# thedonutfactory/zig-tfhe

Measured on AMD Instinct MI355X. Metric: gate-bootstraps/sec (NAND, 128-bit params) at 1/2/4/8 MI355X; % HBM roofline, higher is better.
Workload: dtype f64; 1 GPU; 1024 NAND gate bootstraps per GPU per step, SECURITY_128_BIT (n=700, N=1024, L=3, Bg=2^6, t=9); global_batch=1024, params=128, parallelism=dp1

## Files before the change

include/tfhe_gpu.h:

```cpp
#ifndef TFHE_GPU_H
#define TFHE_GPU_H

#include <stddef.h>
#include <stdint.h>

#ifdef __cplusplus
extern "C" {
#endif

#define TFHE_GPU_ABI_VERSION 7

enum {
    TFHE_OK = 0,
    TFHE_ERR_INVALID = -1,
    TFHE_ERR_HIP = -2,
    TFHE_ERR_NO_KEY = -3,
    TFHE_ERR_OOM = -4,
    TFHE_ERR_IO = -5,
    TFHE_ERR_DEVICE = -6
};

enum {
    TFHE_GATE_NAND = 0, TFHE_GATE_OR = 1, TFHE_GATE_AND = 2, TFHE_GATE_XOR = 3,
    TFHE_GATE_XNOR = 4, TFHE_GATE_NOR = 5, TFHE_GATE_ANDNY = 6, TFHE_GATE_ANDYN = 7,
// ... 44 lines not shown
    TFHE_OPT_KS_NARROW = 4,
    TFHE_OPT_KS_ITEM_GROUPS = 5,
    TFHE_OPT_KS_SEL_ITEMS = 6,
    TFHE_OPT_CIRCUIT_PACK = 7,
    TFHE_OPT_TWIDDLES = 8,
    TFHE_OPT_ARITH = 9,
    TFHE_OPT_BR_SYNC = 10,
    TFHE_OPT_BR_SPIN_CAP = 11,
    TFHE_OPT_HOST_PIPELINE = 12,
    TFHE_OPT_CIRCUIT_SPLIT = 13,
    TFHE_OPT_FUSED_ADMITTED = 14,
    TFHE_OPT_LEVEL_ISSUE_US = 15,
    TFHE_OPT_KEY_ROW_RMS_PPM = 16,
    TFHE_OPT_HOST_STAGING = 17,
    TFHE_OPT_CMUX_FORM = 18,
    TFHE_OPT_PACK_SCRATCH_MB = 19
};
enum { TFHE_STAGING_PAGEABLE = 0, TFHE_STAGING_PINNED = 1 };
enum { TFHE_ARITH_AUTO = 0, TFHE_ARITH_REFERENCE = 1, TFHE_ARITH_FUSED_FORCED = 2 };
enum { TFHE_TWIDDLES_GLIBC = 0, TFHE_TWIDDLES_FDLIBM = 1 };
int tfhe_gpu_set_option(tfhe_gpu_ctx *ctx, int key, int64_t value);
int tfhe_gpu_get_option(const tfhe_gpu_ctx *ctx, int key, int64_t *value);
const char *tfhe_gpu_last_kernels(tfhe_gpu_ctx *ctx);
int tfhe_fft_tables(uint32_t N, int source, double *twist_re, double *twist_im, double *stage_re,
                    double *stage_im);

int tfhe_gpu_load_cloud_key(tfhe_gpu_ctx *ctx, uint32_t decomposition_offset,
                            const uint32_t *testvec_a, const uint32_t *testvec_b,
                            const double *bsk, size_t bsk_len,
                            const uint32_t *ksk, size_t ksk_len);
int tfhe_gpu_keygen(tfhe_gpu_ctx *ctx, uint64_t secret_seed, uint64_t cloud_seed,
// ... 204 lines not shown
```

zig-tfhe_amd/csrc/tfhe_gpu.cpp:

```cpp
#include "tfhe_gpu.h"

#include <algorithm>
#include <cmath>
#include <cstdio>
#include <cstring>
#include <string>
#include <vector>

#include "host_math.hpp"
#include "tfhe_ctx.hpp"

using namespace tfhe;

namespace tfhe {

static thread_local std::string g_create_error;
static int create_fail(int code, const std::string &msg) {
    g_create_error = msg;
    return code;
}

int ensure(Device &d, DevBuf &b, size_t bytes) {
    if (b.bytes >= bytes) return TFHE_OK;
    b.bytes = 0;
// ... 40 lines not shown
    }
    return TFHE_OK;
}

int ks_gemm_args(Device &d, size_t B, KsGemm &G) {
    G = KsGemm();
    if (!ks_use_gemm(d.opts, d.K.iks_t, d.K.basebit, B, nullptr)) return TFHE_OK;
    if (!d.d_ksk_gemm) {
        hipError_t e = hipMalloc((void **)d.d_ksk_gemm.make(d.device), ks_gemm_bytes(d.K, 1024, d.K.iks_t, d.K.basebit));
        if (e != hipSuccess) return fail(d, TFHE_ERR_OOM, "hipMalloc(ksk gemm layout)");
    }
    if (!d.ksk_gemm_ok) {
        HIPCHK(d, launch_ksk_to_gemm(d.K, d.d_ksk, d.d_ksk_gemm, 1024, d.K.iks_t, d.K.basebit, d.stream));
        d.ksk_gemm_ok = true;
    }
    int rc = ensure(d, d.s_kspart, ks_gemm_part_bytes(d.K, B, 1024, d.K.basebit));
    if (rc) return rc;
    G.kg = d.d_ksk_gemm;
    G.part = d.s_kspart.as<uint32_t>();
    return TFHE_OK;
}

static int ensure_tie_flags(Device &d, size_t B) {
    if (d.s_ties.bytes >= B) return TFHE_OK;
    int rc = ensure(d, d.s_ties, B);
    if (rc) return rc;
    HIPCHK(d, hipMemsetAsync(d.s_ties.p, 0, d.s_ties.bytes, d.stream));
    return TFHE_OK;
}

int run_bootstrap_dev(Device &d, const uint8_t *ops, const uint32_t *a, const uint32_t *b,
                      const uint32_t *testvec_dev, uint32_t *out, size_t B, int kind, const uint32_t *idx,
                      const uint32_t *tv_sel) {
    const bool key_switch = kind == RUN_BOOTSTRAP;
// ... 426 lines not shown
    if (!rc) rc = ensure(d, d.s_a, B * wb);
    if (!rc && b) rc = ensure(d, d.s_b, B * wb);
    if (!rc) rc = ensure(d, d.s_out, B * wb);
    if (!rc) rc = ensure(d, d.s_lv1, B * 1025 * sizeof(uint32_t));
    if (!rc) rc = ensure_tie_flags(d, B);
    if (rc) return rc;
    if (!d.pipe_ev) HIPCHK(d, hipEventCreateWithFlags(d.pipe_ev.make(d.device), hipEventDisableTiming));
    for (Stream &p : d.pipe)
        if (!p) HIPCHK(d, hipStreamCreateWithFlags(p.make(d.device), hipStreamNonBlocking));
    if (!d.workers) d.workers.reset(new WorkerPool(PIPE_STREAMS));
    KsGemm G;
    rc = ks_gemm_args(d, chunk, G);
    if (rc) return rc;
    std::vector<KsGemm> Gs(S, G);
    if (G.kg) {
        const size_t pb = ks_gemm_part_bytes(d.K, chunk, 1024, d.K.basebit);
        rc = ensure(d, d.s_kspart, pb * S);
        if (rc) return rc;
        for (int s = 0; s < S; s++) Gs[s].part = (uint32_t *)(d.s_kspart.as<char>() + (size_t)s * pb);
    }
    HIPCHK(d, hipEventRecord(d.pipe_ev, d.stream));
    LaunchOpts o = d.opts;
    if (!o.br_form) o.br_form = 1;
    char *pin_ops = d.pin_in.p, *pin_a = pin_ops + ops_bytes, *pin_b = pin_a + a_bytes;
    uint8_t *d_ops = d.s_ops.as<uint8_t>();
    uint32_t *d_a = d.s_a.as<uint32_t>(), *d_b = d.s_b.as<uint32_t>(), *d_out = d.s_out.as<uint32_t>();
    uint32_t *d_lv1 = d.s_lv1.as<uint32_t>();
    std::vector<hipError_t> err(S, hipSuccess);
    std::vector<const char *> where(S, "");
    d.workers->run(S, [&](int s) {
        hipStream_t st = d.pipe[s];
// ... 125 lines not shown
static int reencrypt_on(Device &d, const tfhe_gpu_reenc_key &key, size_t slot, const uint32_t *in, uint32_t *out,
                        size_t B, bool dev = false) {
    const tfhe_gpu_reenc_key::Copy &k = key.dev[slot];
    if (k.device != d.device) return fail(d, TFHE_ERR_INVALID, "key belongs to another device");
    if (B == 0) return TFHE_OK;
    HIPCHK(d, hipSetDevice(d.device));
    const size_t w = tlwe0_words(d.P);
    Io io{d, dev};
    int rc = ensure(d, d.s_a, B * w * 4 + KS_GEMM_INPUT_SLACK);
    if (!rc) rc = io.out(out, B * w * 4);
    if (rc) return rc;
    if (dev) HIPCHK(d, hipMemcpyAsync(d.s_a.p, in, B * w * 4, hipMemcpyDeviceToDevice, d.stream));
    else if ((rc = h2d(d, d.s_a, in, B * w * 4))) return rc;
    KsGemm G;
    if (k.key_gemm) {
        rc = ensure(d, d.s_kspart, ks_gemm_part_bytes(d.K, B, (int)d.P.n, (int)key.basebit));
        if (rc) return rc;
        G.kg = k.key_gemm;
        G.part = d.s_kspart.as<uint32_t>();
    }
    HIPCHK(d, launch_reencrypt(d.K, (int)key.t, (int)key.basebit, d.s_a.as<const uint32_t>(), k.key, out, B, d.stream,
                               d.opts, &d.last_ks, &G));
    return io.finish();
}

}

extern "C" int tfhe_circuit_schedule(size_t n_inputs, size_t n_gates, const uint8_t *ops, const uint32_t *in_a,
                                     const uint32_t *in_b, uint32_t cus, int pack, uint32_t *levels, uint32_t *depth) {
    if ((n_gates && (!ops || !in_a || !in_b || !levels)) || cus == 0) return TFHE_ERR_INVALID;
    if (n_inputs + n_gates > 0xFFFFFFFFull) return TFHE_ERR_INVALID;
// ... 233 lines not shown
    case TFHE_OPT_BR_SYNC:
        ok = v == 1;
        if (!ok) why = "option " + std::to_string(key) + ": only 1 (the variant with value 0 was removed in round 5)";
        break;
    case TFHE_OPT_KS_NARROW:
    case TFHE_OPT_CIRCUIT_PACK: ok = v == 0 || v == 1; break;
    case TFHE_OPT_KS_ITEM_GROUPS: ok = v == 0 || v == 1 || v == 2 || v == 4 || v == 8; break;
    case TFHE_OPT_KS_SEL_ITEMS: ok = v == 8 || v == 16 || v == 32; break;
    case TFHE_OPT_ARITH: ok = v == TFHE_ARITH_AUTO || v == TFHE_ARITH_REFERENCE || v == TFHE_ARITH_FUSED_FORCED; break;
    case TFHE_OPT_BR_SPIN_CAP: ok = v >= 0 && v <= 0xFFFFFFFFll; break;
    case TFHE_OPT_HOST_PIPELINE: ok = v == 0 || v == 1; break;
    case TFHE_OPT_CIRCUIT_SPLIT: ok = v >= 0 && v <= 2; break;
    case TFHE_OPT_HOST_STAGING: ok = v == TFHE_STAGING_PAGEABLE || v == TFHE_STAGING_PINNED; break;
    case TFHE_OPT_CMUX_FORM: ok = v >= 0 && v <= 2; break;
    case TFHE_OPT_PACK_SCRATCH_MB: ok = v >= 1 && v <= 256; break;
    case TFHE_OPT_TWIDDLES:
        ok = v == TFHE_TWIDDLES_GLIBC || v == TFHE_TWIDDLES_FDLIBM;
        if (ok && d.key_from_keygen && v != d.twiddle_source) {
            why = "TFHE_OPT_TWIDDLES: the resident key was generated (tfhe_gpu_keygen) with the current FFT tables; "
                  "set the twiddle source before keygen";
            return false;
        }
        break;
    default: why = "unknown option key " + std::to_string(key); return false;
    }
    if (!ok && why.empty()) why = "bad value " + std::to_string(v) + " for option " + std::to_string(key);
    return ok;
}

static int apply_option(Device &d, int key, int64_t v) {
// ... 1 lines not shown
    switch (key) {
    case TFHE_OPT_BR_FORM: o.br_form = (int)v; break;
    case TFHE_OPT_BR_LOADER: break;
    case TFHE_OPT_KS_FORM: o.ks_form = (int)v; break;
    case TFHE_OPT_KS_NARROW: o.ks_narrow = (int)v; break;
    case TFHE_OPT_KS_ITEM_GROUPS: o.ks_groups = (int)v; break;
    case TFHE_OPT_KS_SEL_ITEMS: o.ks_sel_items = (int)v; break;
    case TFHE_OPT_CIRCUIT_PACK: d.circuit_pack = v; break;
    case TFHE_OPT_TWIDDLES: return v == d.twiddle_source ? TFHE_OK : build_tables(d, (int)v);
    case TFHE_OPT_BR_SYNC: break;
    case TFHE_OPT_ARITH: o.arith_strict = v == TFHE_ARITH_REFERENCE ? 1 : v == TFHE_ARITH_FUSED_FORCED ? 2 : 0; break;
    case TFHE_OPT_BR_SPIN_CAP: d.K.spin_cap = (uint32_t)v; break;
    case TFHE_OPT_HOST_PIPELINE: d.pipeline = v; break;
    case TFHE_OPT_CMUX_FORM: o.cmux_form = (int)v; break;
    case TFHE_OPT_PACK_SCRATCH_MB: d.pack_scratch_mb = v; break;
    case TFHE_OPT_HOST_STAGING:
        if (d.stage_used) HIPCHK(d, hipStreamSynchronize(d.stream));
        d.stage_used = 0;
        d.host_staging = v;
        break;
    default: return TFHE_ERR_INVALID;
    }
    return TFHE_OK;
}

}

extern "C" {

int tfhe_gpu_set_option(tfhe_gpu_ctx *c, int key, int64_t v) {
// ... 21 lines not shown
    case TFHE_OPT_KS_ITEM_GROUPS: *v = o.ks_groups; break;
    case TFHE_OPT_KS_SEL_ITEMS: *v = o.ks_sel_items; break;
    case TFHE_OPT_CIRCUIT_PACK: *v = d.circuit_pack; break;
    case TFHE_OPT_TWIDDLES: *v = d.twiddle_source; break;
    case TFHE_OPT_ARITH: *v = o.arith_strict == 1 ? TFHE_ARITH_REFERENCE : o.arith_strict == 2 ? TFHE_ARITH_FUSED_FORCED : TFHE_ARITH_AUTO; break;
    case TFHE_OPT_FUSED_ADMITTED: *v = o.key_fused_ok; break;
    case TFHE_OPT_LEVEL_ISSUE_US: *v = c->level_issue_us; break;
    case TFHE_OPT_KEY_ROW_RMS_PPM: *v = (int64_t)std::llround(d.bk_row_rms * 1e6); break;
    case TFHE_OPT_BR_SYNC: *v = 1; break;
    case TFHE_OPT_BR_SPIN_CAP: *v = d.K.spin_cap; break;
    case TFHE_OPT_HOST_PIPELINE: *v = d.pipeline; break;
    case TFHE_OPT_CIRCUIT_SPLIT: *v = c->circuit_split; break;
    case TFHE_OPT_HOST_STAGING: *v = d.host_staging; break;
    case TFHE_OPT_CMUX_FORM: *v = o.cmux_form; break;
    case TFHE_OPT_PACK_SCRATCH_MB: *v = d.pack_scratch_mb; break;
    default: return TFHE_ERR_INVALID;
    }
    return TFHE_OK;
}

const char *tfhe_gpu_last_kernels(tfhe_gpu_ctx *c) {
    if (!c) return "";
    const Device &d = c->dev[0];
    c->last_kernels = d.last_br;
    if (d.last_ks && d.last_ks[0]) c->last_kernels += std::string(" + ") + d.last_ks;
    return c->last_kernels.c_str();
}


int tfhe_gpu_create_multi(const tfhe_params *params, int num_devices, const int *devices, tfhe_gpu_ctx **out) {
// ... 180 lines not shown
```

zig-tfhe_amd/csrc/tfhe_internal.hpp:

```cpp
#pragma once

#include <hip/hip_runtime.h>

#include <cstddef>
#include <cstdint>

namespace tfhe {

struct C2 {
    double x, y;
};

struct KParams {
    int n;
    int N;
    int L;
    int bgbit;
    int basebit;
    int iks_t;
    uint32_t offset;
    int ks_stride;
    uint32_t *err;
    uint32_t spin_cap;
    uint8_t *tie_flags;
// ... 17 lines not shown
    BR_OUT_LV0_EXTRACT2 = 2,
};

struct DevTables {
    const C2 *twist;
    const C2 *tw;
    C2 twa[4];
};

struct LaunchOpts {
    int br_form = 0;
    int ks_form = 3;
    int ks_narrow = 0;
    int ks_groups = 0;
    int ks_sel_items = 8;
    int arith_strict = 0;
    int key_fused_ok = 1;
    int cmux_form = 0;
};
inline bool fused_allowed(const LaunchOpts &O) {
    return O.arith_strict == 2 || (O.arith_strict == 0 && O.key_fused_ok != 0);
}

#if defined(TFHE_PHASE_PROF) && !defined(TFHE_AB_BUILD)
#define TFHE_AB_BUILD 1
#endif
bool kernels_ab_build();
bool ab_forms_linked();

struct BrBatch {
// ... 17 lines not shown
struct BrGeometry {
    dim3 grid, block;
};
BrGeometry br_geometry(char form, size_t B);
hipError_t launch_br(const BrEntry &k, const BrGeometry &g, const KParams &P, const DevTables &T, const BrBatch &b,
                     hipStream_t s, const char **used);
hipError_t launch_blind_rotate(const KParams &P, const DevTables &T, const BrBatch &b, hipStream_t s,
                               const LaunchOpts &O = LaunchOpts(), const char **used = nullptr);
size_t device_cus();
double blind_rotate_cost(size_t B, size_t cus, int L = 3);
hipError_t launch_tlwe_gather(const KParams &P, const uint32_t *src, const uint32_t *idx, uint32_t *dst,
                              size_t count, bool negate, hipStream_t s);
struct KsGemm {
    const uint32_t *kg = nullptr;
    uint32_t *part = nullptr;
};
size_t ks_gemm_bytes(const KParams &P, int n_in, int t, int basebit);
size_t ks_gemm_part_bytes(const KParams &P, size_t B, int n_in, int basebit);
bool ks_gemm_supported(int t, int basebit);
bool ks_use_gemm(const LaunchOpts &O, int t, int basebit, size_t B, const KsGemm *G);
constexpr size_t KS_GEMM_INPUT_SLACK = 16;
hipError_t launch_ksk_to_gemm(const KParams &P, const uint32_t *ksk, uint32_t *kg, int n_in, int t, int basebit,
                              hipStream_t s);
hipError_t launch_key_switch(const KParams &P, const uint32_t *lv1, const uint32_t *ksk,
                             uint32_t *out, size_t B, hipStream_t s, const LaunchOpts &O = LaunchOpts(),
                             const char **used = nullptr, const KsGemm *G = nullptr);
struct PackSums {
    int splits = 0;
    uint32_t bias = 0;
};
size_t pack_gemm_bytes(const KParams &P, int t, int basebit);
size_t pack_gemm_part_bytes(const KParams &P, size_t items, int basebit);
hipError_t launch_pack_key_to_gemm(const KParams &P, const uint32_t *rows, uint32_t *kg, int t, int basebit,
// ... 62 lines not shown
```

zig-tfhe_amd/csrc/tfhe_kernels.hip:

```cpp
#include <algorithm>
#include <string>
#include <type_traits>

#include "tfhe_device.hpp"

namespace tfhe {


constexpr int BO_GATES = 8;
constexpr int BO_LDS_BUF = 2048 * 4;
constexpr int BO_LDS_AT = 1024 * 2;
constexpr int BO_LDS_TOTAL = BR_LDS_BK + BR_LDS_TW + BR_LDS_TWIST + BO_GATES * (BO_LDS_BUF + BO_LDS_AT);
static_assert(BO_LDS_TOTAL <= 160 * 1024, "octo form LDS");
constexpr int BO_LDS_BUF_AT = BR_LDS_BK + BR_LDS_TW + BR_LDS_TWIST;
static_assert(BO_LDS_BUF_AT % 4096 == 0 && BO_LDS_BUF % 4096 == 0, "gather_rot needs 4 KB-aligned buffers");

DEV void issue_bk_pair_async512(const double2 *__restrict__ src, double2 *slot, int tid) {
    const uint32_t base = (uint32_t)(size_t)(lds_void_t *)slot + (uint32_t)(tid & ~63) * 16;
    const uint32_t voff = (uint32_t)tid * 16;
#pragma unroll
    for (int k = 0; k < 4; k++) {
        const uint32_t dst = __builtin_amdgcn_readfirstlane(base + 512 * 16 * k);
        const double2 *piece = src + 512 * k;
        uint32_t keep;
// ... 533 lines not shown
            (w < out_w && i < n_in) ? ksk[((size_t)(base * t) * i + (size_t)base * j + k) * rs + w] : 0u;
        v |= (((word >> (8 * b)) & 255u) ^ 128u) << (8 * e4);
    }
    kg[x] = v;
}

template <int N>
DEV void kg_wait() {
    static_assert(N >= 0 && N <= 15, "kg_wait");
#define KG_W(n_) if constexpr (N == n_) asm volatile("s_waitcnt vmcnt(" #n_ ")" ::: "memory");
    KG_W(0) KG_W(1) KG_W(2) KG_W(3) KG_W(4) KG_W(5) KG_W(6) KG_W(7)
    KG_W(8) KG_W(9) KG_W(10) KG_W(11) KG_W(12) KG_W(13) KG_W(14) KG_W(15)
#undef KG_W
}

template <int T, int BASEBIT>
__global__ __launch_bounds__(64 * KG_WAVES, 1) void k_key_switch_gemm(KParams P, const uint32_t *__restrict__ lv1,
                                                                   const uint32_t *__restrict__ kg,
                                                                   uint32_t *__restrict__ part, size_t B,
                                                                   int ib_per_split, int n_in, int in_stride,
                                                                   int out_w) {
    constexpr int CB = BASEBIT == 2 ? 8 : 4;
    constexpr int KS = BASEBIT == 2 ? 1 : 4;
    constexpr int STEP_BYTES = KS * 4 * 1024;
    constexpr int WORDS_BYTES = CB * KG_ITEMS * 4;
    constexpr int WORD_DMAS = CB / 4;
    constexpr int BUF_BYTES = T * STEP_BYTES + WORDS_BYTES;
    constexpr int STAGES = 3 * BUF_BYTES <= 160 * 1024 ? 3 : 2;
    constexpr int LOADER_DMAS = T * KS + WORD_DMAS;
    constexpr int OTHER_DMAS = WORD_DMAS;
    static_assert(STAGES * BUF_BYTES <= 160 * 1024, "gemm key-switch LDS");
    __shared__ __attribute__((aligned(16))) unsigned char smem[STAGES * BUF_BYTES];
    const int tid = threadIdx.x, lane = tid & 63;
    const int v = __builtin_amdgcn_readfirstlane(tid >> 6);
    const bool loader = v < 4;
    const int w32 = (out_w + 31) / 32;
    const int wt = blockIdx.x;
    const int nib = kg_blocks(n_in, BASEBIT);
    const int ib_lo = blockIdx.z * ib_per_split, ib_hi = min(nib, ib_lo + ib_per_split);
    const size_t m_wg = (size_t)blockIdx.y * KG_ITEMS;
    const int h = lane >> 5, c = lane & 31;
    const uint32_t *a_src[WORD_DMAS];
#pragma unroll
    for (int r = 0; r < WORD_DMAS; r++) {
        const size_t m = m_wg + (CB == 8 ? 256 * r + (tid >> 1) : tid);
        a_src[r] = lv1 + (m < B ? m : B - 1) * (size_t)in_stride + (CB == 8 ? 4 * (tid & 1) : 0);
    }
    const uint32_t lds0 = (uint32_t)(size_t)(lds_void_t *)smem;
    auto issue = [&](int ib, int slot) {
        const uint32_t base = lds0 + slot * BUF_BYTES;
        if (loader) {
#pragma unroll
            for (int j = 0; j < T; j++)
#pragma unroll
                for (int st = 0; st < KS; st++) {
                    const uint32_t *src = kg + ((((size_t)j * nib + ib) * w32 + wt) * KS + st) * 1024 + tid * 4;
                    const uint32_t dst =
                        __builtin_amdgcn_readfirstlane(base + j * STEP_BYTES + st * 4096 + (tid & ~63) * 16);
                    uint32_t keep;
                    asm volatile(
                        "s_mov_b32 %0, m0\n\ts_mov_b32 m0, %2\n\ts_nop 0\n\tglobal_load_lds_dwordx4 %1, off\n\ts_mov_b32 m0, %0"
                        : "=&s"(keep)
                        : "v"(src), "s"(dst)
                        : "memory");
                }
        }
#pragma unroll
        for (int r = 0; r < WORD_DMAS; r++) {
            const uint32_t dst =
                __builtin_amdgcn_readfirstlane(base + T * STEP_BYTES + r * 256 * 32 + (tid & ~63) * 16);
            uint32_t keep;
            asm volatile(
                "s_mov_b32 %0, m0\n\ts_mov_b32 m0, %2\n\ts_nop 0\n\tglobal_load_lds_dwordx4 %1, off\n\ts_mov_b32 m0, %0"
                : "=&s"(keep)
                : "v"(a_src[r] + CB * ib), "s"(dst)
                : "memory");
        }
    };
    kg_v16i acc[2][4];
#pragma unroll
    for (int s = 0; s < 2; s++)
#pragma unroll
        for (int b = 0; b < 4; b++) acc[s][b] = kg_v16i{};
    const uint32_t prec = 1u << (32 - (1 + BASEBIT * T));
#pragma unroll
    for (int k = 0; k < STAGES - 1; k++)
        if (ib_lo + k < ib_hi) issue(ib_lo + k, k);
    for (int ib = ib_lo; ib < ib_hi; ib++) {
        const int slot = (ib - ib_lo) % STAGES;
        const int ahead = min(STAGES - 2, ib_hi - 1 - ib);
        if (ahead == 1) {
            if (loader) kg_wait<LOADER_DMAS>();
            else kg_wait<OTHER_DMAS>();
        } else {
            kg_wait<0>();
        }
        __syncthreads();
        if (ib + STAGES - 1 < ib_hi) issue(ib + STAGES - 1, (slot + STAGES - 1) % STAGES);
        const unsigned char *buf = smem + slot * BUF_BYTES;
        const uint32_t *words = reinterpret_cast<const uint32_t *>(buf + T * STEP_BYTES);
        if constexpr (BASEBIT == 2) {
            uint32_t pk[2][4];
#pragma unroll
            for (int s = 0; s < 2; s++) {
                const kg_v4i wv = *reinterpret_cast<const kg_v4i *>(words + (64 * v + 32 * s + c) * 8 + 4 * h);
#pragma unroll
                for (int q = 0; q < 4; q++) pk[s][q] = ((uint32_t)wv[q] + prec) >> (32 - 2 * T);
            }
#pragma unroll
            for (int j = 0; j < T; j++) {
                kg_v4i a[2];
#pragma unroll
                for (int s = 0; s < 2; s++)
#pragma unroll
                    for (int q = 0; q < 4; q++)
                        a[s][q] = (int)(1u << (8u * ((pk[s][q] >> (2 * (T - 1 - j))) & 3u)));
#pragma unroll
                for (int b = 0; b < 4; b++) {
                    const kg_v4i bf = *reinterpret_cast<const kg_v4i *>(buf + j * STEP_BYTES + b * 1024 + lane * 16);
#pragma unroll
                    for (int s = 0; s < 2; s++)
                        acc[s][b] = __builtin_amdgcn_mfma_i32_32x32x32_i8(a[s], bf, acc[s][b], 0, 0, 0);
                }
            }
        } else {
            uint32_t pk[2][4];
#pragma unroll
            for (int s = 0; s < 2; s++) {
                const kg_v4i wv = *reinterpret_cast<const kg_v4i *>(words + (64 * v + 32 * s + c) * 4);
#pragma unroll
                for (int q = 0; q < 4; q++) pk[s][q] = ((uint32_t)wv[q] + prec) >> (32 - BASEBIT * T);
            }
#pragma unroll
            for (int j = 0; j < T; j++)
#pragma unroll
                for (int st = 0; st < KS; st++) {
                    kg_v4i a[2];
#pragma unroll
// ... 4 lines not shown
#pragma unroll
                        for (int q = 0; q < 4; q++) a[s][q] = word == q ? (int)one : 0;
                    }
#pragma unroll
                    for (int b = 0; b < 4; b++) {
                        const kg_v4i bf = *reinterpret_cast<const kg_v4i *>(buf + j * STEP_BYTES + st * 4096 +
                                                                            b * 1024 + lane * 16);
#pragma unroll
                        for (int s = 0; s < 2; s++)
                            acc[s][b] = __builtin_amdgcn_mfma_i32_32x32x32_i8(a[s], bf, acc[s][b], 0, 0, 0);
                    }
                }
        }
    }
    const int n1 = out_w;
    uint32_t *pz = part + (size_t)blockIdx.z * B * n1;
    const int w = 32 * wt + c;
    const size_t m_base = m_wg + 64 * v;
#pragma unroll
    for (int s = 0; s < 2; s++)
#pragma unroll
        for (int reg = 0; reg < 16; reg++) {
            const size_t m = m_base + 32 * s + (reg & 3) + 8 * (reg >> 2) + 4 * h;
            const uint32_t val = (uint32_t)acc[s][0][reg] + ((uint32_t)acc[s][1][reg] << 8) +
                                 ((uint32_t)acc[s][2][reg] << 16) + ((uint32_t)acc[s][3][reg] << 24);
            if (m < B && w < n1) pz[m * n1 + w] = val;
        }
}

__global__ void k_ks_gemm_reduce(KParams P, const uint32_t *__restrict__ lv1, const uint32_t *__restrict__ part,
                                 uint32_t *__restrict__ out, size_t B, int splits, int n_in, int in_stride, int t,
// ... 662 lines not shown
        }))
        return true;
    if (gw == 4 && basebit == 5 && B > 64)
        return ks_with_shape<KS_GROUPED>(t_, basebit, [&](auto T, auto BB) {
            lanes(dim3(grid.x, (unsigned)((B + 255) / 256)), dim3(256), T, BB, chunk, waves, integral_constant<int, 4>());
        });
    if (gw == 2 && basebit == 5 && B > 64)
        return ks_with_shape<KS_GROUPED>(t_, basebit, [&](auto T, auto BB) {
            lanes(dim3(grid.x, (unsigned)((B + 127) / 128)), dim3(256), T, BB, chunk, waves, integral_constant<int, 2>());
        });
    return ks_with_shape<KS_LANES>(t_, basebit, [&](auto T, auto BB) {
        lanes(grid, block, T, BB, chunk, waves, integral_constant<int, 1>());
    });
}

static int ks_gemm_splits(int out_w, size_t B, int n_in, int basebit) {
    const size_t tiles = (size_t)(out_w + 31) / 32 * ((B + KG_ITEMS - 1) / KG_ITEMS);
    const size_t z = std::max<size_t>(1, device_cus() / tiles);
    return (int)std::min<size_t>(z, (size_t)kg_blocks(n_in, basebit));
}
size_t ks_gemm_part_bytes(const KParams &P, size_t B, int n_in, int basebit) {
    return (size_t)ks_gemm_splits(P.n + 1, B, n_in, basebit) * B * (P.n + 1) * 4;
}

template <bool PACK>
static hipError_t launch_ks_gemm_part(const KParams &P, int t, int basebit, int n_in, int in_stride, int out_w, int z,
                                      const uint32_t *in, const KsGemm &G, size_t B, hipStream_t s, const char **used,
                                      int *splits_out) {
    const int nib = kg_blocks(n_in, basebit);
    const int per = (nib + z - 1) / z;
    const int splits = (nib + per - 1) / per;
    dim3 grid((unsigned)((out_w + 31) / 32), (unsigned)((B + KG_ITEMS - 1) / KG_ITEMS), (unsigned)splits),
        block(64 * KG_WAVES);
    if (!ks_with_shape<KS_GEMM>(t, basebit, [&](auto T, auto BB) {
            hipLaunchKernelGGL((k_key_switch_gemm<T(), BB()>), grid, block, 0, s, P, in, G.kg, G.part, B, per, n_in,
                               in_stride, out_w);
            if (used) *used = ks_name<PACK ? KK_GEMM_PACK : KK_GEMM, T(), BB()>();
        }))
        return hipErrorInvalidValue;
    *splits_out = splits;
    return hipGetLastError();
}

static hipError_t launch_ks_gemm(const KParams &P, int t, int basebit, int n_in, int in_stride, const uint32_t *in,
                                 const KsGemm &G, uint32_t *out, size_t B, hipStream_t s, const char **used) {
    int splits = 0;
    const hipError_t e = launch_ks_gemm_part<false>(P, t, basebit, n_in, in_stride, P.n + 1,
                                                    ks_gemm_splits(P.n + 1, B, n_in, basebit), in, G, B, s, used, &splits);
    if (e != hipSuccess) return e;
    const size_t total = B * (size_t)(P.n + 1);
    hipLaunchKernelGGL(k_ks_gemm_reduce, dim3((unsigned)((total + 255) / 256)), dim3(256), 0, s, P, in, G.part, out, B,
                       splits, n_in, in_stride, t, basebit);
    return hipGetLastError();
}

hipError_t launch_reencrypt(const KParams &P, int t_, int basebit, const uint32_t *in, const uint32_t *key,
                            uint32_t *out, size_t B, hipStream_t s, const LaunchOpts &O, const char **used,
                            const KsGemm *KG) {
    if (B == 0) return hipSuccess;
    if (KG && ks_use_gemm(O, t_, basebit, B, KG))
        return launch_ks_gemm(P, t_, basebit, P.n, P.n + 1, in, *KG, out, B, s, used);
    if (!launch_ks_lanes(P, t_, basebit, in, P.n, P.n + 1, key, out, B, s, O, used)) return hipErrorInvalidValue;
    return hipGetLastError();
}

hipError_t launch_ksk_to_gemm(const KParams &P, const uint32_t *ksk, uint32_t *kg, int n_in, int t, int basebit,
                              hipStream_t s) {
    const size_t words = ks_gemm_bytes(P, n_in, t, basebit) / 4;
    hipLaunchKernelGGL(k_ksk_to_gemm, dim3((unsigned)((words + 255) / 256)), dim3(256), 0, s, P, ksk, kg, words, n_in,
                       t, basebit, P.n + 1, P.ks_stride);
    return hipGetLastError();
}

size_t pack_gemm_bytes(const KParams &P, int t, int basebit) { return ks_gemm_bytes_w(2 * P.N, P.n, t, basebit); }
size_t pack_gemm_part_bytes(const KParams &P, size_t items, int basebit) {
    return (size_t)ks_gemm_splits(2 * P.N, items, P.n, basebit) * items * 2 * P.N * 4;
}
hipError_t launch_pack_key_to_gemm(const KParams &P, const uint32_t *rows, uint32_t *kg, int t, int basebit,
                                   hipStream_t s) {
    const size_t words = pack_gemm_bytes(P, t, basebit) / 4;
    hipLaunchKernelGGL(k_ksk_to_gemm, dim3((unsigned)((words + 255) / 256)), dim3(256), 0, s, P, rows, kg, words, P.n,
                       t, basebit, 2 * P.N, 2 * P.N);
    return hipGetLastError();
}
hipError_t launch_pack_gemm(const KParams &P, int t, int basebit, const uint32_t *in, const KsGemm &G, size_t items,
                            size_t sized_for, hipStream_t s, const char **used, PackSums *sums) {
    if (items > sized_for) return hipErrorInvalidValue;
    sums->bias = (uint32_t)(kg_cb(basebit) * kg_blocks(P.n, basebit) * t) * 128u * 0x01010101u;
    return launch_ks_gemm_part<true>(P, t, basebit, P.n, P.n + 1, 2 * P.N, ks_gemm_splits(2 * P.N, sized_for, P.n, basebit),
                                     in, G, items, s, used, &sums->splits);
}

hipError_t launch_key_switch(const KParams &P, const uint32_t *lv1, const uint32_t *ksk, uint32_t *out,
                             size_t B, hipStream_t s, const LaunchOpts &O, const char **used, const KsGemm *KG) {
    if (B == 0) return hipSuccess;
    if (KG && ks_use_gemm(O, P.iks_t, P.basebit, B, KG))
        return launch_ks_gemm(P, P.iks_t, P.basebit, 1024, 1025, lv1, *KG, out, B, s, used);
    if (O.ks_form != 1 && launch_ks_lanes(P, P.iks_t, P.basebit, lv1, 1024, 1025, ksk, out, B, s, O, used))
        return hipGetLastError();
    if (used) *used = P.basebit == 2 ? "k_key_switch_sel" : "k_key_switch_gather";
    auto with_items = [&](auto f) {
        if (O.ks_sel_items == 16) f(std::integral_constant<int, 16>());
        else if (O.ks_sel_items == 32) f(std::integral_constant<int, 32>());
        else f(std::integral_constant<int, 8>());
    };
    auto launch = [&](auto kernel, int G) {
        dim3 grid((unsigned)((P.n + 1 + 255) / 256), (unsigned)((B + G - 1) / G)), block(256);
        hipLaunchKernelGGL(kernel, grid, block, 0, s, P, lv1, ksk, out, B);
    };
    const bool found =
        P.basebit == 2
            ? ks_with_shape<KS_SEL>(P.iks_t, 2, [&](auto T, auto) {
// ... 147 lines not shown
```

zig-tfhe_amd/csrc/tfhe_pack.cpp:

```cpp
#include "tfhe_gpu.h"

#include <algorithm>
#include <memory>

#include "tfhe_ctx.hpp"

using namespace tfhe;

struct tfhe_gpu_packing_key {
    const tfhe_gpu_ctx *ctx = nullptr;
    tfhe_params P{};
    uint32_t basebit = 0, t = 0;
    DevPtr<uint32_t> key_gemm;
};

namespace tfhe {

static size_t pack_chunk_items(const Device &d, size_t items, int basebit) {
    const size_t cap = (size_t)d.pack_scratch_mb << 20;
    size_t chunk = std::min(items, std::max<size_t>(1, cap / (2 * d.P.N * sizeof(uint32_t))));
    while (chunk > 1 && pack_gemm_part_bytes(d.K, chunk, basebit) > cap) chunk = (chunk + 1) / 2;
    return chunk;
}

// ... 1 lines not shown
                   uint32_t *out, size_t B, bool dev) {
    const size_t items = B * C, w = tlwe0_words(d.P), in_bytes = items * w * sizeof(uint32_t);
    const int basebit = (int)key.basebit, t = (int)key.t;
    Io io{d, dev};
    int rc = ensure(d, d.s_a, in_bytes + 2 * KS_GEMM_INPUT_SLACK);
    if (!rc) rc = io.out(out, B * 2 * d.P.N * sizeof(uint32_t));
    if (!rc) rc = h2d(d, d.s_cidx, coef, C * sizeof(uint32_t));
    if (rc) return rc;
    if (dev) HIPCHK(d, hipMemcpyAsync(d.s_a.p, in, in_bytes, hipMemcpyDeviceToDevice, d.stream));
    else if ((rc = h2d(d, d.s_a, in, in_bytes))) return rc;
    const size_t chunk = pack_chunk_items(d, items, basebit);
    if ((rc = ensure(d, d.s_kspart, pack_gemm_part_bytes(d.K, chunk, basebit)))) return rc;
    KsGemm G;
    G.kg = key.key_gemm;
    G.part = d.s_kspart.as<uint32_t>();
    d.last_br = d.last_ks = "";
    for (size_t item0 = 0; item0 < items; item0 += chunk) {
        const size_t M = std::min(chunk, items - item0);
        const uint32_t *x = d.s_a.as<const uint32_t>() + item0 * w;
        PackSums sums;
        HIPCHK(d, launch_pack_gemm(d.K, t, basebit, x, G, M, chunk, d.stream, &d.last_br, &sums));
        HIPCHK(d, launch_pack_rotate_acc(x, (int)d.P.n, G.part, sums, d.s_cidx.as<const uint32_t>(), C, item0, M, out,
                                         d.stream, &d.last_ks));
    }
    return io.finish();
}

}

extern "C" {
// ... 54 lines not shown
```

zig-tfhe_amd/tfhe_amd.py:

```python
from __future__ import annotations

import contextlib
import ctypes as C
import os
from dataclasses import dataclass

import numpy as np

HERE = os.path.dirname(os.path.abspath(__file__))
LIB_PATH = os.environ.get("TFHE_GPU_LIB") or os.path.join(HERE, "lib", "libtfhe_gpu.so")

OPTIONS = {"br_form": 1, "br_loader": 2, "ks_form": 3, "ks_narrow": 4, "ks_item_groups": 5, "ks_sel_items": 6,
           "circuit_pack": 7, "twiddles": 8, "arith": 9, "br_sync": 10, "br_spin_cap": 11, "host_pipeline": 12,
           "circuit_split": 13, "host_staging": 17, "cmux_form": 18, "pack_scratch_mb": 19}
READONLY_OPTIONS = {"fused_admitted": 14, "level_issue_us": 15, "key_row_rms_ppm": 16}
OPTION_DEFAULTS = {"br_form": 0, "br_loader": 1, "ks_form": 3, "ks_narrow": 0, "ks_item_groups": 0,
                   "ks_sel_items": 8, "circuit_pack": 1, "twiddles": 0, "arith": 0, "br_sync": 1, "br_spin_cap": 0,
                   "host_pipeline": 0, "circuit_split": 0, "host_staging": 0, "cmux_form": 0,
                   "pack_scratch_mb": 256}
ERR_INVALID, ERR_HIP, ERR_NO_KEY, ERR_OOM, ERR_IO, ERR_DEVICE = -1, -2, -3, -4, -5, -6
BR_FORMS = {"auto": 0, "whole": 1, "wide": 3, "octo": 5, "duo": 6, "wide2": 7, "plain": 8}
BUILD_PRODUCT, BUILD_AB = 0, 1
TWIDDLES_GLIBC, TWIDDLES_FDLIBM = 0, 1
ARITH_AUTO, ARITH_REFERENCE, ARITH_FUSED_FORCED = 0, 1, 2
STAGING_PAGEABLE, STAGING_PINNED = 0, 1
CMUX_AUTO, CMUX_PER_WAVE, CMUX_SHARED = 0, 1, 2

NAND, OR, AND, XOR, XNOR, NOR, ANDNY, ANDYN, ORNY, ORYN = range(10)
NOT = 254
COPY = 255
GATE_NAMES = {"nand": NAND, "or": OR, "and": AND, "xor": XOR, "xnor": XNOR, "nor": NOR,
              "andny": ANDNY, "andyn": ANDYN, "orny": ORNY, "oryn": ORYN}


# ... 1483 lines not shown
```

Measured before the change: 168,100 gate-bootstraps/s.

## Restructure GEMM key-switch staging, linearize grid, and software-pipeline MFMA one-hot operands

Reworks the GEMM-form key-switch kernel. Key and input-word LDS buffers are now separate regions, and each wave issues its own word DMAs, so the wait counts match the issue order. The 3D grid becomes a 1D linearized grid in which, for basebit 2, item groups vary fastest so neighbouring workgroups share key tiles in cache. The basebit-2 inner loop double-buffers the B operand reads and computes the next digit's one-hot A operand between MFMAs, with digit masks precomputed. It also adds a ks_gemm_splits option to force the split-K count, which risks extra register pressure and bounds-check complexity.

```diff
diff --git a/include/tfhe_gpu.h b/include/tfhe_gpu.h
--- a/include/tfhe_gpu.h
+++ b/include/tfhe_gpu.h
@@ -82,7 +82,8 @@
     TFHE_OPT_KEY_ROW_RMS_PPM = 16,
     TFHE_OPT_HOST_STAGING = 17,
     TFHE_OPT_CMUX_FORM = 18,
-    TFHE_OPT_PACK_SCRATCH_MB = 19
+    TFHE_OPT_PACK_SCRATCH_MB = 19,
+    TFHE_OPT_KS_GEMM_SPLITS = 20
 };
 enum { TFHE_STAGING_PAGEABLE = 0, TFHE_STAGING_PINNED = 1 };
 enum { TFHE_ARITH_AUTO = 0, TFHE_ARITH_REFERENCE = 1, TFHE_ARITH_FUSED_FORCED = 2 };
diff --git a/zig-tfhe_amd/csrc/tfhe_gpu.cpp b/zig-tfhe_amd/csrc/tfhe_gpu.cpp
--- a/zig-tfhe_amd/csrc/tfhe_gpu.cpp
+++ b/zig-tfhe_amd/csrc/tfhe_gpu.cpp
@@ -78,10 +78,12 @@
         HIPCHK(d, launch_ksk_to_gemm(d.K, d.d_ksk, d.d_ksk_gemm, 1024, d.K.iks_t, d.K.basebit, d.stream));
         d.ksk_gemm_ok = true;
     }
-    int rc = ensure(d, d.s_kspart, ks_gemm_part_bytes(d.K, B, 1024, d.K.basebit));
+    const size_t pb = ks_gemm_part_bytes(d.K, B, 1024, d.K.basebit, d.opts.ks_gemm_splits);
+    int rc = ensure(d, d.s_kspart, pb);
     if (rc) return rc;
     G.kg = d.d_ksk_gemm;
     G.part = d.s_kspart.as<uint32_t>();
+    G.part_bytes = pb;
     return TFHE_OK;
 }
 
@@ -538,7 +540,7 @@
     if (rc) return rc;
     std::vector<KsGemm> Gs(S, G);
     if (G.kg) {
-        const size_t pb = ks_gemm_part_bytes(d.K, chunk, 1024, d.K.basebit);
+        const size_t pb = G.part_bytes;
         rc = ensure(d, d.s_kspart, pb * S);
         if (rc) return rc;
         for (int s = 0; s < S; s++) Gs[s].part = (uint32_t *)(d.s_kspart.as<char>() + (size_t)s * pb);
@@ -694,7 +696,10 @@
     else if ((rc = h2d(d, d.s_a, in, B * w * 4))) return rc;
     KsGemm G;
     if (k.key_gemm) {
-        rc = ensure(d, d.s_kspart, ks_gemm_part_bytes(d.K, B, (int)d.P.n, (int)key.basebit));
+        if (d.opts.ks_gemm_splits > ks_gemm_blocks((int)d.P.n, (int)key.basebit))
+            return fail(d, TFHE_ERR_INVALID, "ks_gemm_splits above the key's coefficient blocks");
+        G.part_bytes = ks_gemm_part_bytes(d.K, B, (int)d.P.n, (int)key.basebit, d.opts.ks_gemm_splits);
+        rc = ensure(d, d.s_kspart, G.part_bytes);
         if (rc) return rc;
         G.kg = k.key_gemm;
         G.part = d.s_kspart.as<uint32_t>();
@@ -958,6 +963,11 @@
     case TFHE_OPT_HOST_STAGING: ok = v == TFHE_STAGING_PAGEABLE || v == TFHE_STAGING_PINNED; break;
     case TFHE_OPT_CMUX_FORM: ok = v >= 0 && v <= 2; break;
     case TFHE_OPT_PACK_SCRATCH_MB: ok = v >= 1 && v <= 256; break;
+    case TFHE_OPT_KS_GEMM_SPLITS:
+        ok = v >= 0 && v <= ks_gemm_blocks(1024, d.K.basebit);
+        if (!ok) why = "TFHE_OPT_KS_GEMM_SPLITS: 0 (auto) or 1 .. " + std::to_string(ks_gemm_blocks(1024, d.K.basebit)) +
+                       ", the key switch's coefficient blocks";
+        break;
     case TFHE_OPT_TWIDDLES:
         ok = v == TFHE_TWIDDLES_GLIBC || v == TFHE_TWIDDLES_FDLIBM;
         if (ok && d.key_from_keygen && v != d.twiddle_source) {
@@ -989,6 +999,7 @@
     case TFHE_OPT_HOST_PIPELINE: d.pipeline = v; break;
     case TFHE_OPT_CMUX_FORM: o.cmux_form = (int)v; break;
     case TFHE_OPT_PACK_SCRATCH_MB: d.pack_scratch_mb = v; break;
+    case TFHE_OPT_KS_GEMM_SPLITS: o.ks_gemm_splits = (int)v; break;
     case TFHE_OPT_HOST_STAGING:
         if (d.stage_used) HIPCHK(d, hipStreamSynchronize(d.stream));
         d.stage_used = 0;
@@ -1040,6 +1051,7 @@
     case TFHE_OPT_HOST_STAGING: *v = d.host_staging; break;
     case TFHE_OPT_CMUX_FORM: *v = o.cmux_form; break;
     case TFHE_OPT_PACK_SCRATCH_MB: *v = d.pack_scratch_mb; break;
+    case TFHE_OPT_KS_GEMM_SPLITS: *v = o.ks_gemm_splits; break;
     default: return TFHE_ERR_INVALID;
     }
     return TFHE_OK;
diff --git a/zig-tfhe_amd/csrc/tfhe_internal.hpp b/zig-tfhe_amd/csrc/tfhe_internal.hpp
--- a/zig-tfhe_amd/csrc/tfhe_internal.hpp
+++ b/zig-tfhe_amd/csrc/tfhe_internal.hpp
@@ -55,6 +55,7 @@
     int ks_narrow = 0;
     int ks_groups = 0;
     int ks_sel_items = 8;
+    int ks_gemm_splits = 0;
     int arith_strict = 0;
     int key_fused_ok = 1;
     int cmux_form = 0;
@@ -102,9 +103,11 @@
 struct KsGemm {
     const uint32_t *kg = nullptr;
     uint32_t *part = nullptr;
+    size_t part_bytes = 0;
 };
 size_t ks_gemm_bytes(const KParams &P, int n_in, int t, int basebit);
-size_t ks_gemm_part_bytes(const KParams &P, size_t B, int n_in, int basebit);
+size_t ks_gemm_part_bytes(const KParams &P, size_t B, int n_in, int basebit, int splits = 0);
+int ks_gemm_blocks(int n_in, int basebit);
 bool ks_gemm_supported(int t, int basebit);
 bool ks_use_gemm(const LaunchOpts &O, int t, int basebit, size_t B, const KsGemm *G);
 constexpr size_t KS_GEMM_INPUT_SLACK = 16;
diff --git a/zig-tfhe_amd/csrc/tfhe_kernels.hip b/zig-tfhe_amd/csrc/tfhe_kernels.hip
--- a/zig-tfhe_amd/csrc/tfhe_kernels.hip
+++ b/zig-tfhe_amd/csrc/tfhe_kernels.hip
@@ -571,68 +571,81 @@
 #undef KG_W
 }
 
+DEV void kg_dma(const uint32_t *src, uint32_t dst) {
+    uint32_t keep;
+    asm volatile("s_mov_b32 %0, m0\n\ts_mov_b32 m0, %2\n\ts_nop 0\n\tglobal_load_lds_dwordx4 %1, off\n\ts_mov_b32 m0, %0"
+                 : "=&s"(keep)
+                 : "v"(src), "s"(dst)
+                 : "memory");
+}
+
+template <int T, int BASEBIT>
+struct KgIssue {
+    static constexpr int CB = BASEBIT == 2 ? 8 : 4;
+    static constexpr int KS = BASEBIT == 2 ? 1 : 4;
+    static constexpr int STEPS = T * KS;
+    static constexpr int WORD_DMAS = CB / 4;
+    static constexpr int key_dmas(bool loader) { return loader ? STEPS : 0; }
+    static constexpr bool GROUP_FASTEST = BASEBIT == 2;
+    static constexpr int STEP_BYTES = KS * 4 * 1024;
+    static constexpr int KEY_BYTES = T * STEP_BYTES;
+    static constexpr int WORDS_BYTES = CB * KG_ITEMS * 4;
+    static constexpr int STAGES = 3 * (KEY_BYTES + WORDS_BYTES) <= 160 * 1024 ? 3 : 2;
+    static constexpr int LDS_BYTES = STAGES * (KEY_BYTES + WORDS_BYTES);
+    static constexpr int ahead_dmas(bool loader) { return STAGES == 3 ? WORD_DMAS + key_dmas(loader) : 0; }
+    static_assert(LDS_BYTES <= 160 * 1024, "gemm key-switch LDS");
+    static_assert(ahead_dmas(true) <= 15, "vmcnt immediate");
+};
+
 template <int T, int BASEBIT>
 __global__ __launch_bounds__(64 * KG_WAVES, 1) void k_key_switch_gemm(KParams P, const uint32_t *__restrict__ lv1,
                                                                    const uint32_t *__restrict__ kg,
                                                                    uint32_t *__restrict__ part, size_t B,
                                                                    int ib_per_split, int n_in, int in_stride,
                                                                    int out_w) {
-    constexpr int CB = BASEBIT == 2 ? 8 : 4;
-    constexpr int KS = BASEBIT == 2 ? 1 : 4;
-    constexpr int STEP_BYTES = KS * 4 * 1024;
-    constexpr int WORDS_BYTES = CB * KG_ITEMS * 4;
-    constexpr int WORD_DMAS = CB / 4;
-    constexpr int BUF_BYTES = T * STEP_BYTES + WORDS_BYTES;
-    constexpr int STAGES = 3 * BUF_BYTES <= 160 * 1024 ? 3 : 2;
-    constexpr int LOADER_DMAS = T * KS + WORD_DMAS;
-    constexpr int OTHER_DMAS = WORD_DMAS;
-    static_assert(STAGES * BUF_BYTES <= 160 * 1024, "gemm key-switch LDS");
-    __shared__ __attribute__((aligned(16))) unsigned char smem[STAGES * BUF_BYTES];
+    using I = KgIssue<T, BASEBIT>;
+    constexpr int CB = I::CB, KS = I::KS, STEP_BYTES = I::STEP_BYTES, KEY_BYTES = I::KEY_BYTES;
+    constexpr int WORDS_BYTES = I::WORDS_BYTES, WORD_DMAS = I::WORD_DMAS;
+    constexpr int STAGES = I::STAGES;
+    __shared__ __attribute__((aligned(16))) unsigned char smem[I::LDS_BYTES];
     const int tid = threadIdx.x, lane = tid & 63;
     const int v = __builtin_amdgcn_readfirstlane(tid >> 6);
     const bool loader = v < 4;
     const int w32 = (out_w + 31) / 32;
-    const int wt = blockIdx.x;
     const int nib = kg_blocks(n_in, BASEBIT);
-    const int ib_lo = blockIdx.z * ib_per_split, ib_hi = min(nib, ib_lo + ib_per_split);
-    const size_t m_wg = (size_t)blockIdx.y * KG_ITEMS;
+    const unsigned groups = (unsigned)((B + KG_ITEMS - 1) / KG_ITEMS), lin = blockIdx.x;
+    const unsigned fast = I::GROUP_FASTEST ? groups : (unsigned)w32, slow = I::GROUP_FASTEST ? (unsigned)w32 : groups;
+    const int wt = (int)(I::GROUP_FASTEST ? lin / fast % slow : lin % fast);
+    const int grp = (int)(I::GROUP_FASTEST ? lin % fast : lin / fast % slow);
+    const int split = (int)(lin / fast / slow);
+    const int ib_lo = split * ib_per_split, ib_hi = min(nib, ib_lo + ib_per_split);
+    const size_t m_wg = (size_t)grp * KG_ITEMS;
     const int h = lane >> 5, c = lane & 31;
     const uint32_t *a_src[WORD_DMAS];
 #pragma unroll
     for (int r = 0; r < WORD_DMAS; r++) {
-        const size_t m = m_wg + (CB == 8 ? 256 * r + (tid >> 1) : tid);
-        a_src[r] = lv1 + (m < B ? m : B - 1) * (size_t)in_stride + (CB == 8 ? 4 * (tid & 1) : 0);
+        const size_t m = m_wg + 64 * v + (CB == 8 ? 32 * r + (lane >> 1) : lane);
+        a_src[r] = lv1 + (m < B ? m : B - 1) * (size_t)in_stride + (CB == 8 ? 4 * (lane & 1) : 0);
     }
     const uint32_t lds0 = (uint32_t)(size_t)(lds_void_t *)smem;
-    auto issue = [&](int ib, int slot) {
-        const uint32_t base = lds0 + slot * BUF_BYTES;
-        if (loader) {
-#pragma unroll
-            for (int j = 0; j < T; j++)
-#pragma unroll
-                for (int st = 0; st < KS; st++) {
-                    const uint32_t *src = kg + ((((size_t)j * nib + ib) * w32 + wt) * KS + st) * 1024 + tid * 4;
-                    const uint32_t dst =
-                        __builtin_amdgcn_readfirstlane(base + j * STEP_BYTES + st * 4096 + (tid & ~63) * 16);
-                    uint32_t keep;
-                    asm volatile(
-                        "s_mov_b32 %0, m0\n\ts_mov_b32 m0, %2\n\ts_nop 0\n\tglobal_load_lds_dwordx4 %1, off\n\ts_mov_b32 m0, %0"
-                        : "=&s"(keep)
-                        : "v"(src), "s"(dst)
-                        : "memory");
-                }
-        }
-#pragma unroll
-        for (int r = 0; r < WORD_DMAS; r++) {
-            const uint32_t dst =
-                __builtin_amdgcn_readfirstlane(base + T * STEP_BYTES + r * 256 * 32 + (tid & ~63) * 16);
-            uint32_t keep;
-            asm volatile(
-                "s_mov_b32 %0, m0\n\ts_mov_b32 m0, %2\n\ts_nop 0\n\tglobal_load_lds_dwordx4 %1, off\n\ts_mov_b32 m0, %0"
-                : "=&s"(keep)
-                : "v"(a_src[r] + CB * ib), "s"(dst)
-                : "memory");
-        }
+    const uint32_t ldsw = lds0 + STAGES * KEY_BYTES;
+    const uint32_t *key_src = kg + ((size_t)wt * KS) * 1024 + (tid & 255) * 4;
+    const size_t level_words = (size_t)nib * w32 * KS * 1024, block_words = (size_t)w32 * KS * 1024;
+    auto issue_keys = [&](int ib, int slot) {
+        if (!loader) return;
+        const uint32_t base = lds0 + slot * KEY_BYTES + (v & 3) * 1024;
+        const uint32_t *src = key_src + ib * block_words;
+#pragma unroll
+        for (int p = 0; p < I::key_dmas(true); p++) {
+            const int j = p / KS, st = p % KS;
+            kg_dma(src + j * level_words + st * 1024, __builtin_amdgcn_readfirstlane(base + j * STEP_BYTES + st * 4096));
+        }
+    };
+    auto issue_words = [&](int ib, int slot) {
+#pragma unroll
+        for (int r = 0; r < WORD_DMAS; r++)
+            kg_dma(a_src[r] + CB * ib,
+                   __builtin_amdgcn_readfirstlane(ldsw + slot * WORDS_BYTES + (64 * v) * (CB * 4) + r * 1024));
     };
     kg_v16i acc[2][4];
 #pragma unroll
@@ -640,45 +653,62 @@
 #pragma unroll
         for (int b = 0; b < 4; b++) acc[s][b] = kg_v16i{};
     const uint32_t prec = 1u << (32 - (1 + BASEBIT * T));
+    auto issue = [&](int ib, int slot) {
+        issue_words(ib, slot);
+        issue_keys(ib, slot);
+    };
 #pragma unroll
     for (int k = 0; k < STAGES - 1; k++)
         if (ib_lo + k < ib_hi) issue(ib_lo + k, k);
     for (int ib = ib_lo; ib < ib_hi; ib++) {
         const int slot = (ib - ib_lo) % STAGES;
-        const int ahead = min(STAGES - 2, ib_hi - 1 - ib);
-        if (ahead == 1) {
-            if (loader) kg_wait<LOADER_DMAS>();
-            else kg_wait<OTHER_DMAS>();
+        if (STAGES == 3 && ib + 1 < ib_hi) {
+            if (loader) kg_wait<I::ahead_dmas(true)>();
+            else kg_wait<I::ahead_dmas(false)>();
         } else {
             kg_wait<0>();
         }
         __syncthreads();
         if (ib + STAGES - 1 < ib_hi) issue(ib + STAGES - 1, (slot + STAGES - 1) % STAGES);
-        const unsigned char *buf = smem + slot * BUF_BYTES;
-        const uint32_t *words = reinterpret_cast<const uint32_t *>(buf + T * STEP_BYTES);
+        const unsigned char *buf = smem + slot * KEY_BYTES;
+        const uint32_t *words = reinterpret_cast<const uint32_t *>(smem + STAGES * KEY_BYTES + slot * WORDS_BYTES);
         if constexpr (BASEBIT == 2) {
-            uint32_t pk[2][4];
+            uint32_t pk[2][4][3];
 #pragma unroll
             for (int s = 0; s < 2; s++) {
                 const kg_v4i wv = *reinterpret_cast<const kg_v4i *>(words + (64 * v + 32 * s + c) * 8 + 4 * h);
 #pragma unroll
-                for (int q = 0; q < 4; q++) pk[s][q] = ((uint32_t)wv[q] + prec) >> (32 - 2 * T);
+                for (int q = 0; q < 4; q++)
+#pragma unroll
+                    for (int m3 = 0; m3 < 3; m3++) {
+                        uint32_t mask = 0;
+                        for (int j = m3; j < T; j += 3) mask |= 3u << (30 - 2 * j);
+                        pk[s][q][m3] = ((uint32_t)wv[q] + prec) & mask;
+                        asm("" : "+v"(pk[s][q][m3]));
+                    }
             }
+            kg_v4i a[2][2], bf[2][4];
+            auto read_b = [&](int j) {
+#pragma unroll
+                for (int b = 0; b < 4; b++)
+                    bf[j & 1][b] = *reinterpret_cast<const kg_v4i *>(buf + j * STEP_BYTES + b * 1024 + lane * 16);
+            };
+            auto one_hot = [&](int j, int s, int q) {
+                a[j & 1][s][q] = (int)(1u << ((pk[s][q][j % 3] >> (27 - 2 * j)) & 31u));
+            };
+            read_b(0);
+#pragma unroll
+            for (int x = 0; x < 8; x++) one_hot(0, x >> 2, x & 3);
 #pragma unroll
             for (int j = 0; j < T; j++) {
-                kg_v4i a[2];
-#pragma unroll
-                for (int s = 0; s < 2; s++)
-#pragma unroll
-                    for (int q = 0; q < 4; q++)
-                        a[s][q] = (int)(1u << (8u * ((pk[s][q] >> (2 * (T - 1 - j))) & 3u)));
-#pragma unroll
-                for (int b = 0; b < 4; b++) {
-                    const kg_v4i bf = *reinterpret_cast<const kg_v4i *>(buf + j * STEP_BYTES + b * 1024 + lane * 16);
-#pragma unroll
-                    for (int s = 0; s < 2; s++)
-                        acc[s][b] = __builtin_amdgcn_mfma_i32_32x32x32_i8(a[s], bf, acc[s][b], 0, 0, 0);
-                }
+                if (j + 1 < T) read_b(j + 1);
+#pragma unroll
+                for (int b = 0; b < 4; b++)
+#pragma unroll
+                    for (int s = 0; s < 2; s++) {
+                        acc[s][b] = __builtin_amdgcn_mfma_i32_32x32x32_i8(a[j & 1][s], bf[j & 1][b], acc[s][b], 0, 0, 0);
+                        if (j + 1 < T) one_hot(j + 1, (2 * b + s) >> 2, (2 * b + s) & 3);
+                    }
             }
         } else {
             uint32_t pk[2][4];
@@ -713,7 +743,7 @@
         }
     }
     const int n1 = out_w;
-    uint32_t *pz = part + (size_t)blockIdx.z * B * n1;
+    uint32_t *pz = part + (size_t)split * B * n1;
     const int w = 32 * wt + c;
     const size_t m_base = m_wg + 64 * v;
 #pragma unroll
@@ -1406,13 +1436,16 @@
     });
 }
 
-static int ks_gemm_splits(int out_w, size_t B, int n_in, int basebit) {
+static int ks_gemm_splits(int out_w, size_t B, int n_in, int basebit, int forced) {
+    const int nib = kg_blocks(n_in, basebit);
+    if (forced) return forced <= nib ? forced : 0;
     const size_t tiles = (size_t)(out_w + 31) / 32 * ((B + KG_ITEMS - 1) / KG_ITEMS);
     const size_t z = std::max<size_t>(1, device_cus() / tiles);
-    return (int)std::min<size_t>(z, (size_t)kg_blocks(n_in, basebit));
-}
-size_t ks_gemm_part_bytes(const KParams &P, size_t B, int n_in, int basebit) {
-    return (size_t)ks_gemm_splits(P.n + 1, B, n_in, basebit) * B * (P.n + 1) * 4;
+    return (int)std::min<size_t>(z, (size_t)nib);
+}
+int ks_gemm_blocks(int n_in, int basebit) { return kg_blocks(n_in, basebit); }
+size_t ks_gemm_part_bytes(const KParams &P, size_t B, int n_in, int basebit, int forced) {
+    return (size_t)ks_gemm_splits(P.n + 1, B, n_in, basebit, forced) * B * (P.n + 1) * 4;
 }
 
 template <bool PACK>
@@ -1420,10 +1453,13 @@
                                       const uint32_t *in, const KsGemm &G, size_t B, hipStream_t s, const char **used,
                                       int *splits_out) {
     const int nib = kg_blocks(n_in, basebit);
+    if (z < 1 || z > nib) return hipErrorInvalidValue;
     const int per = (nib + z - 1) / z;
     const int splits = (nib + per - 1) / per;
-    dim3 grid((unsigned)((out_w + 31) / 32), (unsigned)((B + KG_ITEMS - 1) / KG_ITEMS), (unsigned)splits),
-        block(64 * KG_WAVES);
+    if ((size_t)splits * B * (size_t)out_w * 4 > G.part_bytes) return hipErrorInvalidValue;
+    const size_t wgs = (size_t)((out_w + 31) / 32) * ((B + KG_ITEMS - 1) / KG_ITEMS) * (size_t)splits;
+    if (wgs > 0x7fffffffu) return hipErrorInvalidValue;
+    dim3 grid((unsigned)wgs), block(64 * KG_WAVES);
     if (!ks_with_shape<KS_GEMM>(t, basebit, [&](auto T, auto BB) {
             hipLaunchKernelGGL((k_key_switch_gemm<T(), BB()>), grid, block, 0, s, P, in, G.kg, G.part, B, per, n_in,
                                in_stride, out_w);
@@ -1435,10 +1471,12 @@
 }
 
 static hipError_t launch_ks_gemm(const KParams &P, int t, int basebit, int n_in, int in_stride, const uint32_t *in,
-                                 const KsGemm &G, uint32_t *out, size_t B, hipStream_t s, const char **used) {
+                                 const KsGemm &G, uint32_t *out, size_t B, hipStream_t s, const LaunchOpts &O,
+                                 const char **used) {
     int splits = 0;
-    const hipError_t e = launch_ks_gemm_part<false>(P, t, basebit, n_in, in_stride, P.n + 1,
-                                                    ks_gemm_splits(P.n + 1, B, n_in, basebit), in, G, B, s, used, &splits);
+    const hipError_t e =
+        launch_ks_gemm_part<false>(P, t, basebit, n_in, in_stride, P.n + 1,
+                                   ks_gemm_splits(P.n + 1, B, n_in, basebit, O.ks_gemm_splits), in, G, B, s, used, &splits);
     if (e != hipSuccess) return e;
     const size_t total = B * (size_t)(P.n + 1);
     hipLaunchKernelGGL(k_ks_gemm_reduce, dim3((unsigned)((total + 255) / 256)), dim3(256), 0, s, P, in, G.part, out, B,
@@ -1451,7 +1489,7 @@
                             const KsGemm *KG) {
     if (B == 0) return hipSuccess;
     if (KG && ks_use_gemm(O, t_, basebit, B, KG))
-        return launch_ks_gemm(P, t_, basebit, P.n, P.n + 1, in, *KG, out, B, s, used);
+        return launch_ks_gemm(P, t_, basebit, P.n, P.n + 1, in, *KG, out, B, s, O, used);
     if (!launch_ks_lanes(P, t_, basebit, in, P.n, P.n + 1, key, out, B, s, O, used)) return hipErrorInvalidValue;
     return hipGetLastError();
 }
@@ -1466,7 +1504,7 @@
 
 size_t pack_gemm_bytes(const KParams &P, int t, int basebit) { return ks_gemm_bytes_w(2 * P.N, P.n, t, basebit); }
 size_t pack_gemm_part_bytes(const KParams &P, size_t items, int basebit) {
-    return (size_t)ks_gemm_splits(2 * P.N, items, P.n, basebit) * items * 2 * P.N * 4;
+    return (size_t)ks_gemm_splits(2 * P.N, items, P.n, basebit, 0) * items * 2 * P.N * 4;
 }
 hipError_t launch_pack_key_to_gemm(const KParams &P, const uint32_t *rows, uint32_t *kg, int t, int basebit,
                                    hipStream_t s) {
@@ -1479,7 +1517,7 @@
                             size_t sized_for, hipStream_t s, const char **used, PackSums *sums) {
     if (items > sized_for) return hipErrorInvalidValue;
     sums->bias = (uint32_t)(kg_cb(basebit) * kg_blocks(P.n, basebit) * t) * 128u * 0x01010101u;
-    return launch_ks_gemm_part<true>(P, t, basebit, P.n, P.n + 1, 2 * P.N, ks_gemm_splits(2 * P.N, sized_for, P.n, basebit),
+    return launch_ks_gemm_part<true>(P, t, basebit, P.n, P.n + 1, 2 * P.N, ks_gemm_splits(2 * P.N, sized_for, P.n, basebit, 0),
                                      in, G, items, s, used, &sums->splits);
 }
 
@@ -1487,7 +1525,7 @@
                              size_t B, hipStream_t s, const LaunchOpts &O, const char **used, const KsGemm *KG) {
     if (B == 0) return hipSuccess;
     if (KG && ks_use_gemm(O, P.iks_t, P.basebit, B, KG))
-        return launch_ks_gemm(P, P.iks_t, P.basebit, 1024, 1025, lv1, *KG, out, B, s, used);
+        return launch_ks_gemm(P, P.iks_t, P.basebit, 1024, 1025, lv1, *KG, out, B, s, O, used);
     if (O.ks_form != 1 && launch_ks_lanes(P, P.iks_t, P.basebit, lv1, 1024, 1025, ksk, out, B, s, O, used))
         return hipGetLastError();
     if (used) *used = P.basebit == 2 ? "k_key_switch_sel" : "k_key_switch_gather";
diff --git a/zig-tfhe_amd/csrc/tfhe_pack.cpp b/zig-tfhe_amd/csrc/tfhe_pack.cpp
--- a/zig-tfhe_amd/csrc/tfhe_pack.cpp
+++ b/zig-tfhe_amd/csrc/tfhe_pack.cpp
@@ -39,6 +39,7 @@
     KsGemm G;
     G.kg = key.key_gemm;
     G.part = d.s_kspart.as<uint32_t>();
+    G.part_bytes = pack_gemm_part_bytes(d.K, chunk, basebit);
     d.last_br = d.last_ks = "";
     for (size_t item0 = 0; item0 < items; item0 += chunk) {
         const size_t M = std::min(chunk, items - item0);
diff --git a/zig-tfhe_amd/tfhe_amd.py b/zig-tfhe_amd/tfhe_amd.py
--- a/zig-tfhe_amd/tfhe_amd.py
+++ b/zig-tfhe_amd/tfhe_amd.py
@@ -12,12 +12,13 @@
 
 OPTIONS = {"br_form": 1, "br_loader": 2, "ks_form": 3, "ks_narrow": 4, "ks_item_groups": 5, "ks_sel_items": 6,
            "circuit_pack": 7, "twiddles": 8, "arith": 9, "br_sync": 10, "br_spin_cap": 11, "host_pipeline": 12,
-           "circuit_split": 13, "host_staging": 17, "cmux_form": 18, "pack_scratch_mb": 19}
+           "circuit_split": 13, "host_staging": 17, "cmux_form": 18, "pack_scratch_mb": 19,
+           "ks_gemm_splits": 20}
 READONLY_OPTIONS = {"fused_admitted": 14, "level_issue_us": 15, "key_row_rms_ppm": 16}
 OPTION_DEFAULTS = {"br_form": 0, "br_loader": 1, "ks_form": 3, "ks_narrow": 0, "ks_item_groups": 0,
                    "ks_sel_items": 8, "circuit_pack": 1, "twiddles": 0, "arith": 0, "br_sync": 1, "br_spin_cap": 0,
                    "host_pipeline": 0, "circuit_split": 0, "host_staging": 0, "cmux_form": 0,
-                   "pack_scratch_mb": 256}
+                   "pack_scratch_mb": 256, "ks_gemm_splits": 0}
 ERR_INVALID, ERR_HIP, ERR_NO_KEY, ERR_OOM, ERR_IO, ERR_DEVICE = -1, -2, -3, -4, -5, -6
 BR_FORMS = {"auto": 0, "whole": 1, "wide": 3, "octo": 5, "duo": 6, "wide2": 7, "plain": 8}
 BUILD_PRODUCT, BUILD_AB = 0, 1
```

Result: no change. 168,100 gate-bootstraps/s, median of 3 (-0.0%).
